# gopro/cineform-sdk

Measured on AMD Instinct MI355X. Metric: 1080p YUY2 encode+decode fps, higher is better.
Workload: dtype int16

## Files before the change

cineform-sdk_amd/csrc/cfhd_kernels.h:

```cpp
#pragma once
#include <stdint.h>
#include <cfhd_gfx950.h>

namespace cfhd {
namespace dev {

enum { TW = 64, TH = 16, ROWS = 2 * TH + 4, NTHREADS = 256, NSTAGE = (ROWS * (TW + 4) + NTHREADS - 1) / NTHREADS };

struct QuantParam { int mid; unsigned mult; int divisor; };

struct FwdPlaneJob {
	const int16_t *in; int in_pitch;
	int width, height;
	int prescale;
	int16_t *out[4]; int out_pitch;
	QuantParam q[4];
	int xstride, shift, display_height;
	int compand;
	int layout, tail_from;
	const uint16_t *curve;
};
enum FwdLayout { FWD_WORDS16 = 0, FWD_V210_Y = 1, FWD_V210_CR = 2, FWD_V210_CB = 3, FWD_BYTES8_BOTTOM_UP = 4, FWD_BYTES8_TOP_DOWN = 5, FWD_RGB10 = 6, FWD_RGB16_AS_422 = 7,
                 FWD_BYTES8_AS_422_BOTTOM_UP = 8, FWD_BYTES8_AS_422_TOP_DOWN = 9, FWD_BAYER_BYR4 = 10, FWD_BAYER_BYR5 = 11,
                 FWD_AVID_BYTES8 = 12, FWD_AVID_WORDS16 = 13, FWD_AVID_S214 = 14, FWD_AVID_2_8 = 15 };
static_assert(FWD_V210_CB < FWD_BYTES8_BOTTOM_UP && FWD_BYTES8_TOP_DOWN < FWD_RGB10 && FWD_RGB10 < FWD_RGB16_AS_422 && FWD_RGB16_AS_422 < FWD_BYTES8_AS_422_BOTTOM_UP &&
              FWD_BYTES8_AS_422_TOP_DOWN < FWD_BAYER_BYR4 && FWD_BAYER_BYR5 == 11 && FWD_BAYER_BYR5 < FWD_AVID_BYTES8 && FWD_AVID_2_8 == 15,
              "fwd_plane_tile's loader tests the pairs as ranges");

__device__ __forceinline__ uint32_t rgb16_to_yuv_sample(const uint16_t *p, int wpp, int which, int color_space, int x)
{
	const int m[4][10] = { { 2998, 10060, 1016, 64, 1655, 5538, 7193, 7193, 6537, 655 }, { 3490, 11715, 1180, 0, 1917, 6455, 8372, 8372, 7602, 770 },
	                       { 4211, 8258, 1606, 64, 2425, 4768, 7193, 7193, 6029, 1163 }, { 4899, 9617, 1868, 0, 2818, 5554, 8372, 8372, 7012, 1360 } };
	const int cs = color_space & 3;
	if (which == 0) {
		const uint16_t *q = p + (size_t)x * wpp;
		const int y = ((m[cs][0] * (int)q[0] + m[cs][1] * (int)q[1] + m[cs][2] * (int)q[2]) >> 20) + m[cs][3];
		return (uint32_t)(y < 0 ? 0 : (y > 1023 ? 1023 : y));
	}
	int acc = 0;
#pragma unroll
	for (int k = 0; k < 2; k++) {
		const uint16_t *q = p + (size_t)(2 * x + k) * wpp;
		const int r = q[0], g = q[1], b = q[2];
		acc += which == 2 ? (-m[cs][4] * r - m[cs][5] * g + m[cs][6] * b) >> 20 : (m[cs][7] * r - m[cs][8] * g - m[cs][9] * b) >> 20;
	}
	acc = (acc >> 1) + 512;
	return (uint32_t)(acc < 0 ? 0 : (acc > 1023 ? 1023 : acc));
}

__device__ __forceinline__ uint32_t rgb8_to_yuv_sample(const uint8_t *row, int bpp, int which, int color_space, int x)
{
	const int m[4][9] = { { 1499, 5029, 507, 827, 2768, 3596, 3596, 3268, 327 }, { 1744, 5857, 589, 958, 3227, 4186, 4186, 3801, 385 },
	                      { 2105, 4128, 802, 1212, 2383, 3596, 3596, 3014, 581 }, { 2449, 4808, 933, 1409, 2777, 4186, 4186, 3506, 679 } };
	const int cs = color_space & 3;
	const uint8_t *q = row + (size_t)(which ? 2 * x : x) * bpp;
	const int b = (int)q[0] << 7, g = (int)q[1] << 7, r = (int)q[2] << 7;
	int v;
	if (which == 0) v = ((((m[cs][0] * r) >> 16) + ((m[cs][1] * g) >> 16) + ((m[cs][2] * b) >> 16)) << 2) + ((cs & 1) ? 0 : 1024);
	else if (which == 2) v = ((((-m[cs][3] * r) >> 16) + ((-m[cs][4] * g) >> 16) + ((m[cs][5] * b) >> 16)) * 4) + 8192;
	else v = ((((m[cs][6] * r) >> 16) + ((-m[cs][7] * g) >> 16) + ((-m[cs][8] * b) >> 16)) * 4) + 8192;
	v = v < 0 ? 0 : (v > 16383 ? 16383 : v);
	return (uint32_t)v >> 4;
}

__device__ __forceinline__ uint32_t bayer_plane_sample(const FwdPlaneJob &job, int row, int x)
{
	int tl, tr, bl, br;
	if (job.layout == FWD_BAYER_BYR5) {
		const uint8_t *base = (const uint8_t *)job.in + (size_t)row * job.width * 6, *nib = base + (size_t)job.width * 4;
		int v[4];
#pragma unroll
		for (int k = 0; k < 4; k++) { const int s = k * job.width + x; v[k] = ((int)base[s] << 4) | ((nib[s >> 1] >> (4 * (s & 1))) & 15); }
		tl = v[0]; tr = v[1]; bl = v[2]; br = v[3];
	} else {
		const uint16_t *l1 = (const uint16_t *)job.in + (size_t)(2 * row) * job.in_pitch, *l2 = l1 + job.in_pitch;
		const uint32_t a = *(const uint32_t *)(l1 + 2 * x), b = *(const uint32_t *)(l2 + 2 * x);
		tl = job.curve[(a & 0xffffu) >> 2]; tr = job.curve[a >> 18]; bl = job.curve[(b & 0xffffu) >> 2]; br = job.curve[b >> 18];
	}
	int r, g1, g2, bb;
	switch (job.xstride) {
	case 0: r = tl; g1 = tr; g2 = bl; bb = br; break;
	case 1: g1 = tl; r = tr; bb = bl; g2 = br; break;
	case 3: bb = tl; g1 = tr; g2 = bl; r = br; break;
	default: g1 = tl; bb = tr; r = bl; g2 = br; break;
	}
	const int mid = 1 << (job.shift - 1), g = (g1 + g2) >> 1;
	const int v = job.tail_from == 0 ? g : (job.tail_from == 1 ? ((r - g) >> 1) + mid : (job.tail_from == 2 ? ((bb - g) >> 1) + mid : (g1 - g2 + 2 * mid) >> 1));
	return (uint32_t)(uint16_t)v;
}

__device__ __forceinline__ uint32_t avid_sample(const FwdPlaneJob &job, int y, int s)
{
	const uint8_t *frame = (const uint8_t *)job.in;
	if (job.layout == FWD_AVID_BYTES8) return (uint32_t)frame[(size_t)y * job.in_pitch + s] << 2;
	if (job.layout == FWD_AVID_2_8) {
		const uint32_t upper = frame[(size_t)y * (job.in_pitch >> 2) + (s >> 2)], lower = frame[(size_t)job.shift + (size_t)y * job.in_pitch + s];
		return (lower << 2) | ((upper >> (6 - 2 * (s & 3))) & 3u);
	}
	const uint32_t w = *(const uint16_t *)(frame + (size_t)y * job.in_pitch + 2 * (size_t)s);
	if (job.layout == FWD_AVID_WORDS16) return w >> 6;
	const int v = (int)(int16_t)w;
	const int n = job.tail_from == 1 ? 219 * v : 224 * (v + 8192);
	const int q = (((n + ((n >> 31) & 16383)) >> 14) + 16) * 4;
	return (uint32_t)(q < 0 ? 0 : (q > 1023 ? 1023 : q));
}

enum { FWD_CHUNK_BLOCKS = 62, FWD_CHUNK_COLS = FWD_CHUNK_BLOCKS * 8 };
struct FwdBlockLists {
	uint4 *blocks;
	unsigned long long *masks;
	const int16_t *base;
	int mask_base[3][4];
	int reserved[2];
};

struct FwdYuvJob {
	const uint8_t *in; int in_pitch;
	int width, height, display_height;
	int uyvy, shift;
	int16_t *out[3][4]; int out_pitch[3];
	QuantParam q[3][4];
	FwdBlockLists lists;
};

struct InvPlaneJob {
	const int16_t *band[4]; int band_pitch;
	int width, height;
	int descale;
	int16_t *out; int out_pitch;
	int xstride, precision, display_height;
	int alpha;
	int alpha_const;
	int bytes8, bottom_up;
	uint32_t dither_seed;
	int bit_shift, big_endian;
	int ll_bottom_row_high;
};

struct InvYuvJob {
	const int16_t *band[3][4]; int band_pitch[3];
	int width, height;
	int display_height;
	int uyvy, shift;
	uint32_t dither_seed;
	uint8_t *out; int out_pitch;
	int bottom_up, matrix_601;
	const unsigned long long *masks; int mask_base[3][4];
};

struct HalfYuvJob {
	const int16_t *ll[3]; int pitch[3];
	int width, rows;
	int uyvy;
	uint8_t *out; int out_pitch;
	int matrix;
	int mode, bottom_up;
};

struct HalfPackedJob {
	const int16_t *ll[4]; int pitch;
	int width, rows, nch;
	int word[4];
	int shift, alpha;
	uint16_t *out; int out_pitch;
	int mode, bytes, bottom_up, big_endian; uint32_t dither_seed;
};

struct FwdFrameJob {
	const uint8_t *in; int in_pitch;
	int width, height, display_height;
	int uyvy, shift;
	int16_t *out[3][4]; int out_pitch[3];
	QuantParam q[3][4];
	FwdBlockLists lists;
};

struct BayerJob {
	const uint16_t *in; int in_pitch;
	int width, height, display_height;
	int16_t *out[4]; int out_pitch;
	const uint16_t *curve;
	int order;
	int precision;
	int packed12;
};

__device__ __forceinline__ int sat16(int x) { return x < -32768 ? -32768 : (x > 32767 ? 32767 : x); }
__device__ __forceinline__ int adds16(int a, int b) { return sat16(a + b); }
__device__ __forceinline__ int subs16(int a, int b) { return sat16(a - b); }
__device__ __forceinline__ int lo16(uint32_t v) { return (int)(int16_t)(v & 0xffffu); }
__device__ __forceinline__ int hi16(uint32_t v) { return (int)(int16_t)(v >> 16); }
__device__ __forceinline__ uint32_t pack16(int lo, int hi) { return ((uint32_t)(uint16_t)lo) | ((uint32_t)(uint16_t)hi << 16); }

__device__ __forceinline__ uint32_t pk_set(int v) { return pack16(v, v); }
__device__ __forceinline__ uint32_t pk_hp_mid(uint32_t a0, uint32_t a1, uint32_t a2, uint32_t a3, uint32_t a4, uint32_t a5)
{
	uint32_t s = pk_subs(0u, a0);
	s = pk_subs(s, a1);
	s = pk_adds(s, a4);
	s = pk_adds(s, a5);
	s = pk_adds(s, pk_set(4));
	s = pk_sra(s, 3);
	return pk_adds(s, pk_subs(a2, a3));
}

__device__ __forceinline__ int quantize(int v, const QuantParam &q)
{
	if (q.divisor <= 1) return v;
	int neg = v < 0;
	unsigned a = ((unsigned)(neg ? -v : v) + (unsigned)q.mid) & 0xffffu;
	int r = (int)((a * (q.mult & 0xffffu)) >> 16);
	return (int)(int16_t)(neg ? -r : r);
}

__device__ __forceinline__ uint32_t pk_quantize(uint32_t v, const QuantParam &q)
{
	if (q.divisor <= 1) return v;
	const uint32_t s = pk_sra(v, 15);
	uint32_t a = pk_maxs(v, pk_negw(v));
	a = pk_addw(a, pk_set(q.mid));
	const uint32_t m = q.mult & 0xffffu;
	const uint32_t r = pk_hihi((a & 0xffffu) * m, (a >> 16) * m);
	return pk_addw(r ^ s, pk_negw(s));
}

__device__ __forceinline__ QuantParam wave_uniform_quant(const QuantParam &q) { QuantParam u; u.mid = wave_uniform(q.mid); u.mult = (unsigned)wave_uniform((int)q.mult); u.divisor = wave_uniform(q.divisor); return u; }

__device__ __forceinline__ int hp_mid(int a0, int a1, int a2, int a3, int a4, int a5)
{
	int s = subs16(0, a0);
	s = subs16(s, a1);
	s = adds16(s, a4);
	s = adds16(s, a5);
	s = adds16(s, 4);
	s >>= 3;
	return adds16(s, subs16(a2, a3));
}
__device__ __forceinline__ int hp_first(int a0, int a1, int a2, int a3, int a4, int a5) { return sat16((5 * a0 - 11 * a1 + 4 * a2 + 4 * a3 - a4 - a5 + 4) >> 3); }
__device__ __forceinline__ int hp_last(int a0, int a1, int a2, int a3, int a4, int a5) { return sat16((11 * a4 - 5 * a5 - 4 * a3 - 4 * a2 + a1 + a0 + 4) >> 3); }

__device__ __forceinline__ void horiz_pair(const uint32_t *d, uint32_t dm2, int prescale, bool first0, bool last0, bool last1, uint32_t &lpk, uint32_t &hpk)
{
	uint32_t p0 = d[0], p1 = d[1], p2 = d[2], p3 = d[3];
	if (prescale) {
		const uint32_t three = pk_set(3);
		p0 = pk_adds(p0, three); p1 = pk_adds(p1, three); p2 = pk_adds(p2, three); p3 = pk_adds(p3, three);
		uint32_t low = pk_adds(pk_lolo(p1, p2), pk_hihi(p1, p2));
		low = pk_subs(low, three);
		lpk = pk_sra(low, 2);
		p0 = pk_sra(p0, 2); p1 = pk_sra(p1, 2); p2 = pk_sra(p2, 2); p3 = pk_sra(p3, 2);
	} else {
		lpk = pk_adds(pk_lolo(p1, p2), pk_hihi(p1, p2));
	}
	const uint32_t em = pk_lolo(p0, p1), om = pk_hihi(p0, p1), e0 = pk_lolo(p1, p2), o0 = pk_hihi(p1, p2), ep = pk_lolo(p2, p3), op = pk_hihi(p2, p3);
	hpk = pk_hp_mid(em, om, e0, o0, ep, op);
	if (first0 || last0 || last1) {
		int h0 = lo16(hpk), h1 = hi16(hpk);
		if (first0) h0 = hp_first(lo16(p1), hi16(p1), lo16(p2), hi16(p2), lo16(p3), hi16(p3));
		if (last0) {
			uint32_t pm = dm2;
			if (prescale) pm = pk_sra(pk_adds(pm, pk_set(3)), 2);
			h0 = hp_last(lo16(pm), hi16(pm), lo16(p0), hi16(p0), lo16(p1), hi16(p1));
		}
		if (last1) h1 = hp_last(lo16(p0), hi16(p0), lo16(p1), hi16(p1), lo16(p2), hi16(p2));
		hpk = pack16(h0, h1);
	}
}

__device__ __forceinline__ void vert_pair_store(const uint32_t *sl, const uint32_t *sh, int stride, int pos, const QuantParam *q,
                                                int16_t *const *out, int out_pitch, int r, int c, bool valid1)
{
	uint32_t L[6], H[6];
#pragma unroll
	for (int k = 0; k < 6; k++) { L[k] = sl[k * stride]; H[k] = sh[k * stride]; }
	uint32_t ll, hl, lh, hh;
	if (pos == 1) {
		ll = pk_adds(L[2], L[3]); hl = pk_hp_mid(L[0], L[1], L[2], L[3], L[4], L[5]);
		lh = pk_adds(H[2], H[3]); hh = pk_hp_mid(H[0], H[1], H[2], H[3], H[4], H[5]);
	} else {
		int res[4][2];
#pragma unroll
		for (int e = 0; e < 2; e++) {
			int a[6], b[6];
#pragma unroll
			for (int k = 0; k < 6; k++) { a[k] = e ? hi16(L[k]) : lo16(L[k]); b[k] = e ? hi16(H[k]) : lo16(H[k]); }
			if (pos == 0) {
				res[0][e] = sat16(a[0] + a[1]); res[2][e] = hp_first(a[0], a[1], a[2], a[3], a[4], a[5]);
				res[1][e] = sat16(b[0] + b[1]); res[3][e] = hp_first(b[0], b[1], b[2], b[3], b[4], b[5]);
			} else {
				res[0][e] = sat16(a[4] + a[5]); res[2][e] = hp_last(a[0], a[1], a[2], a[3], a[4], a[5]);
				res[1][e] = sat16(b[4] + b[5]); res[3][e] = hp_last(b[0], b[1], b[2], b[3], b[4], b[5]);
			}
		}
		ll = pack16(res[0][0], res[0][1]); lh = pack16(res[1][0], res[1][1]); hl = pack16(res[2][0], res[2][1]); hh = pack16(res[3][0], res[3][1]);
	}
	lh = pack16(quantize(lo16(lh), q[1]), quantize(hi16(lh), q[1]));
	hl = pack16(quantize(lo16(hl), q[2]), quantize(hi16(hl), q[2]));
	hh = pack16(quantize(lo16(hh), q[3]), quantize(hi16(hh), q[3]));
	if (!valid1) { ll &= 0xffffu; lh &= 0xffffu; hl &= 0xffffu; hh &= 0xffffu; }
	const size_t o = (size_t)r * out_pitch + c;
	*(uint32_t *)(out[0] + o) = ll; *(uint32_t *)(out[1] + o) = lh; *(uint32_t *)(out[2] + o) = hl; *(uint32_t *)(out[3] + o) = hh;
}

template <typename J> __device__ __forceinline__ void stage_job(J *dst, const J *src)
{
// ... 766 lines not shown
	const int seg_first = tile.x * SSEG;
	const int base = luma ? seg_first + SLUMA_STEP * wave : seg_first >> 1;
	const int want = base - 1 + lane;
	const int blk = want < 0 ? 0 : (want < nblk ? want : nblk - 1);
	const bool stores = lane >= 1 && lane <= SLUMA_STEP && want < nblk;
	const int v_base = SSEG * 4, u_base = v_base + SSEG * 2;
	const int lds_at = luma ? 4 * (want - seg_first) : (comp == 1 ? v_base : u_base) + 4 * (want - (seg_first >> 1));
	const int seg_blocks = job.width / SBLK - seg_first < SSEG ? job.width / SBLK - seg_first : SSEG;
	const int nquads = 2 * seg_blocks;
	const bool first = blk == 0, last = blk == nblk - 1;
	const int pitch = job.band_pitch[comp];
	const int16_t *const bLL = wave_uniform_ptr(job.band[comp][0]), *const bLH = wave_uniform_ptr(job.band[comp][1]);
	const int16_t *const bHL = wave_uniform_ptr(job.band[comp][2]), *const bHH = wave_uniform_ptr(job.band[comp][3]);
	const uint32_t boff = (uint32_t)(SBLK * blk);
#define pLL (bLL + boff)
#define pLH (bLH + boff)
#define pHL (bHL + boff)
#define pHH (bHH + boff)
	if (r0 >= h) return;
	const int nrows = h - r0 < ROWS_PER_STRIP ? h - r0 : ROWS_PER_STRIP;
	int j = inv_window_first_row(r0, h);
	const unsigned long long *const mLH = BLOCKS ? wave_uniform_ptr(job.masks + job.mask_base[comp][1]) : nullptr;
	const unsigned long long *const mHL = BLOCKS ? wave_uniform_ptr(job.masks + job.mask_base[comp][2]) : nullptr;
	const unsigned long long *const mHH = BLOCKS ? wave_uniform_ptr(job.masks + job.mask_base[comp][3]) : nullptr;
	const uint32_t pitch8 = (uint32_t)pitch / SBLK;
#define LOAD_LH(row) (BLOCKS ? strip_load_listed(bLH, mLH, (uint32_t)(row) * pitch8 + (uint32_t)blk) : strip_load(pLH + (size_t)(row) * pitch))
#define LOAD_HL(row) (BLOCKS ? strip_load_listed(bHL, mHL, (uint32_t)(row) * pitch8 + (uint32_t)blk) : strip_load(pHL + (size_t)(row) * pitch))
#define LOAD_HH(row) (BLOCKS ? strip_load_listed(bHH, mHH, (uint32_t)(row) * pitch8 + (uint32_t)blk) : strip_load(pHH + (size_t)(row) * pitch))
	StripRow ll0 = strip_load(pLL + (size_t)j * pitch), ll1 = strip_load(pLL + (size_t)(j + 1) * pitch), ll2 = strip_load(pLL + (size_t)(j + 2) * pitch);
	StripRow lh0 = LOAD_LH(j), lh1 = LOAD_LH(j + 1), lh2 = LOAD_LH(j + 2);
	StripRow hl = LOAD_HL(r0), hh = LOAD_HH(r0);
	const int sh = job.shift;
	uint8_t *const out_base = wave_uniform_ptr(job.out);
	const int out_pitch = wave_uniform(job.out_pitch), display_height = wave_uniform(job.display_height), uyvy = wave_uniform(job.uyvy);
	const int dgroup = luma ? (blk & ~1) : 2 * blk + 1;
	const uint32_t drot = (luma ? (blk & 1) != 0 : comp == 2) ? 8u : 0u;
	for (int s = 0; s < nrows; s++) {
		const int r = r0 + s;
		const bool more = s + 1 < nrows;
		const int jn = more ? inv_window_first_row(r + 1, h) : j;
		const bool advance = jn != j;
		StripRow nll = ll2, nlh = lh2, nhl = hl, nhh = hh;
		if (!LATE_LOADS) {
			if (advance) { nll = strip_load(pLL + (size_t)(jn + 2) * pitch); nlh = LOAD_LH(jn + 2); }
			if (more) { nhl = LOAD_HL(r + 1); nhh = LOAD_HH(r + 1); }
		}
		const int pos = r == 0 ? 0 : (r == h - 1 ? 2 : 1);
		uint32_t Lv[2][4], Hv[2][4];
		if (pos == 1) {
#pragma unroll
			for (int d = 0; d < 4; d++) {
				inv_vert_pk(ll0.d[d], ll1.d[d], ll2.d[d], hl.d[d], 1, Lv[0][d], Lv[1][d]);
				inv_vert_pk(lh0.d[d], lh1.d[d], lh2.d[d], hh.d[d], 1, Hv[0][d], Hv[1][d]);
			}
		} else {
#pragma unroll
			for (int d = 0; d < 4; d++) {
				inv_vert_pk(ll0.d[d], ll1.d[d], ll2.d[d], hl.d[d], pos, Lv[0][d], Lv[1][d]);
				inv_vert_pk(lh0.d[d], lh1.d[d], lh2.d[d], hh.d[d], pos, Hv[0][d], Hv[1][d]);
			}
		}
		uint32_t (*rowbuf)[SROW / 4] = s_rows[s & 1];
#pragma unroll
		for (int par = 0; par < 2; par++) {
			const int orow = 2 * r + par;
			const uint32_t prev = __shfl(Lv[par][3], lane - 1), next = __shfl(Lv[par][0], lane + 1);
			const uint32_t X = sh >= 2 ? rotr32(dither_word(seed, orow, dgroup), drot) : 0u;
			uint32_t out[4];
			strip_row_to8(Lv[par], Hv[par], prev, next, first, last, sh + 1, X, out);
			if (stores) {
				uint32_t *dst = &rowbuf[par][lds_at];
#pragma unroll
				for (int d = 0; d < 4; d++) dst[d] = out[d];
			}
		}
		__syncthreads();
		if (tid < nquads) {
#pragma unroll
			for (int par = 0; par < 2; par++) {
				const int orow = 2 * r + par;
				if (orow >= display_height) continue;
				const uint32_t *row = rowbuf[par];
				const uint32_t y0 = row[2 * tid], y1 = row[2 * tid + 1], vv = row[v_base + tid], uu = row[u_base + tid];
				const uint32_t uv01 = byte_perm(vv, uu, 0x05010400u), uv23 = byte_perm(vv, uu, 0x07030602u);
				uint4 q;
				if (uyvy) {
					q.x = byte_perm(uv01, y0, 0x01050004u); q.y = byte_perm(uv01, y0, 0x03070206u);
					q.z = byte_perm(uv23, y1, 0x01050004u); q.w = byte_perm(uv23, y1, 0x03070206u);
				} else {
					q.x = byte_perm(uv01, y0, 0x05010400u); q.y = byte_perm(uv01, y0, 0x07030602u);
					q.z = byte_perm(uv23, y1, 0x05010400u); q.w = byte_perm(uv23, y1, 0x07030602u);
				}
				*(uint4 *)(out_base + (size_t)orow * out_pitch + 32 * (size_t)seg_first + 16 * (size_t)tid) = q;
			}
		}
		if (LATE_LOADS) {
			if (advance) { nll = strip_load(pLL + (size_t)(jn + 2) * pitch); nlh = LOAD_LH(jn + 2); }
			if (more) { nhl = LOAD_HL(r + 1); nhh = LOAD_HH(r + 1); }
		}
		if (advance) { ll0 = ll1; ll1 = ll2; ll2 = nll; lh0 = lh1; lh1 = lh2; lh2 = nlh; j = jn; }
		hl = nhl; hh = nhh;
	}
#undef pLL
#undef pLH
#undef pHL
#undef pHH
#undef LOAD_LH
#undef LOAD_HL
#undef LOAD_HH
}
__global__ void __launch_bounds__(NTHREADS) k_inv_yuv422_strip(const InvYuvJob *jobs, uint32_t launch_seed) { inv_yuv422_strip<SR, true>(jobs, launch_seed); }
__global__ void __launch_bounds__(NTHREADS) k_inv_yuv422_strip_blocks(const InvYuvJob *jobs, uint32_t launch_seed) { inv_yuv422_strip<SR, true, true>(jobs, launch_seed); }

enum { SRF = 32, SFPLANE = 512 };

__device__ __forceinline__ void strip_fwd_row(const uint32_t (&p)[8], uint32_t prev, uint32_t next, bool first, bool last, uint32_t (&L)[4], uint32_t (&H)[4], int prescale = 0)
{
	const uint32_t ext[10] = { prev, p[0], p[1], p[2], p[3], p[4], p[5], p[6], p[7], next };
#pragma unroll
	for (int m = 0; m < 4; m++) horiz_pair(&ext[2 * m], 0u, prescale, first && m == 0, false, last && m == 3, L[m], H[m]);
}

enum { FWD_LATE_LOADS = 2 };
struct FwdStrip {
	uint32_t LW[6][4], HW[6][4];
	cfhd_u4 raw[2][2];
};

__device__ __forceinline__ void strip_fwd_fetch(FwdStrip &st, const FwdYuvJob &job, const uint8_t *in, int y)
{
#pragma unroll
	for (int k = 0; k < 2; k++) {
		if (y + k < job.display_height) { const uint8_t *p = in + (size_t)(y + k) * job.in_pitch; st.raw[k][0] = CFHD_LDG128(p); st.raw[k][1] = CFHD_LDG128(p + 16); }
		else { cfhd_u4 g; g.x = g.y = g.z = g.w = 0x80808080u; st.raw[k][0] = g; st.raw[k][1] = g; }
	}
}

template <int SLOT>
__device__ __forceinline__ void strip_fwd_push(FwdStrip &st, const FwdYuvJob &job, const uint8_t *in, uint32_t (*buf)[2][SFPLANE], int y, bool prefetch,
                                               bool luma, int comp, int lds_write_at, int lds_read_at, int lane, bool first, bool last, int shift, int ysh0, uint32_t usel, uint32_t vsel)
{
	uint32_t p[2][8];
	if (luma) {
		if (FWD_LATE_LOADS == 2) strip_fwd_fetch(st, job, in, y);
		uint32_t a[2][8];
#pragma unroll
		for (int k = 0; k < 2; k++) {
			a[k][0] = st.raw[k][0].x; a[k][1] = st.raw[k][0].y; a[k][2] = st.raw[k][0].z; a[k][3] = st.raw[k][0].w;
			a[k][4] = st.raw[k][1].x; a[k][5] = st.raw[k][1].y; a[k][6] = st.raw[k][1].z; a[k][7] = st.raw[k][1].w;
		}
		if (prefetch && !FWD_LATE_LOADS) strip_fwd_fetch(st, job, in, y + 2);
#pragma unroll
		for (int k = 0; k < 2; k++) {
#pragma unroll
			for (int i = 0; i < 8; i++) p[k][i] = ((a[k][i] >> ysh0) & 0x00ff00ffu) << shift;
			if (lds_write_at >= 0) {
#pragma unroll
				for (int i = 0; i < 4; i++) {
					buf[k][0][lds_write_at + i] = byte_perm(a[k][2 * i + 1], a[k][2 * i], vsel) << shift;
					buf[k][1][lds_write_at + i] = byte_perm(a[k][2 * i + 1], a[k][2 * i], usel) << shift;
				}
			}
		}
	}
	__syncthreads();
	if (!luma) {
#pragma unroll
		for (int k = 0; k < 2; k++) {
#pragma unroll
			for (int i = 0; i < 8; i++) p[k][i] = buf[k][comp - 1][lds_read_at + i < 0 ? 0 : lds_read_at + i];
		}
	}
#pragma unroll
	for (int k = 0; k < 2; k++) {
		const uint32_t prev = __shfl(p[k][7], lane - 1), next = __shfl(p[k][0], lane + 1);
		strip_fwd_row(p[k], prev, next, first, last, st.LW[SLOT + k], st.HW[SLOT + k]);
	}
	if (luma && prefetch && FWD_LATE_LOADS == 1) strip_fwd_fetch(st, job, in, y + 2);
}

template <int ROWS_PER_STRIP, bool BLOCKS = false, bool DENSE = true>
__device__ __forceinline__ void fwd_yuv422_strip(const FwdYuvJob *jobs)
{
	const TileId tile = xcd_tile();
	__shared__ FwdYuvJob s_job;
	stage_job(&s_job, &jobs[tile.z]);
	const FwdYuvJob &job = s_job;
	__shared__ uint32_t s_pairs[2][2][2][SFPLANE];
	const int W = job.width, H = job.height, HH = H >> 1;
	const int r0 = tile.y * ROWS_PER_STRIP;
	const int tid = threadIdx.x, wave = tid >> 6, lane = tid & 63;
	const bool luma = wave < 2;
	const int comp = luma ? 0 : wave - 1;
	const QuantParam q_lh = wave_uniform_quant(job.q[comp][1]), q_hl = wave_uniform_quant(job.q[comp][2]), q_hh = wave_uniform_quant(job.q[comp][3]);
	const int nblk = luma ? W / 16 : W / 32;
	const int seg_first = tile.x * SSEG;
	const int base = luma ? seg_first + SLUMA_STEP * wave : seg_first >> 1;
	const int want = base - 1 + lane;
	const int blk = want < 0 ? 0 : (want < nblk ? want : nblk - 1);
	const bool stores = lane >= 1 && lane <= SLUMA_STEP && want < nblk;
	const bool first = blk == 0, last = blk == nblk - 1;
	const int lds_write_at = (luma && want >= 0 && want < nblk && (wave == 0 ? lane <= SLUMA_STEP : lane >= 1)) ? 4 * (want - seg_first + 1) : -1;
	const int lds_read_at = 8 * lane - 4;
	if (r0 >= HH) return;
	const int r1 = r0 + ROWS_PER_STRIP < HH ? r0 + ROWS_PER_STRIP : HH;
	const int shift = job.shift;
	const int ysh0 = job.uyvy ? 8 : 0, ub = job.uyvy ? 0 : 1, vb = job.uyvy ? 2 : 3;
	const uint32_t usel = (uint32_t)ub | 0x0c00u | ((uint32_t)(4 + ub) << 16) | 0x0c000000u;
	const uint32_t vsel = (uint32_t)vb | 0x0c00u | ((uint32_t)(4 + vb) << 16) | 0x0c000000u;
	const uint8_t *in = job.in + 32 * (size_t)blk;
	static_assert(SLUMA_STEP == FWD_CHUNK_BLOCKS, "a chunk is what one wave stores of a band row");
	const int chunks_per_row = BLOCKS ? wave_uniform((nblk + FWD_CHUNK_BLOCKS - 1) / FWD_CHUNK_BLOCKS) : 0, chunk = BLOCKS ? wave_uniform(base / FWD_CHUNK_BLOCKS) : 0;
	uint4 *slot0[3]; unsigned long long *mask0[3];
	const int opitch = wave_uniform(job.out_pitch[comp]), pitch8 = opitch >> 3;
	int16_t *outp[4];
#pragma unroll
	for (int b = 0; b < 4; b++) outp[b] = wave_uniform_ptr(job.out[comp][b]);
	if (BLOCKS) {
#pragma unroll
		for (int b = 1; b < 4; b++) {
			slot0[b - 1] = wave_uniform_ptr(job.lists.blocks + (size_t)(job.out[comp][b] - job.lists.base) / 8 + (size_t)(FWD_CHUNK_BLOCKS * chunk));
			mask0[b - 1] = wave_uniform_ptr(job.lists.masks + job.lists.mask_base[comp][b] + chunk);
		}
	}
	FwdStrip st;
	int wtop = window_first_row(r0, HH, H);
	const int lastrow = window_first_row(r1 - 1, HH, H) + 5;
	int t = 0;
#define CFHD_PUSH(SLOT, Y) strip_fwd_push<SLOT>(st, job, in, s_pairs[t & 1], (Y), (Y) + 2 <= lastrow, luma, comp, lds_write_at, lds_read_at, lane, first, last, shift, ysh0, usel, vsel); t++
	if (luma && FWD_LATE_LOADS != 2) strip_fwd_fetch(st, job, in, wtop);
	CFHD_PUSH(0, wtop); CFHD_PUSH(2, wtop + 2); CFHD_PUSH(4, wtop + 4);
	auto band_row = [&](const int r, const int pos) {
		uint32_t o[4][4];
#pragma unroll
		for (int d = 0; d < 4; d++) {
			uint32_t ll, lh, hl, hh;
			if (pos == 1) {
				ll = pk_adds(st.LW[2][d], st.LW[3][d]); hl = pk_hp_mid(st.LW[0][d], st.LW[1][d], st.LW[2][d], st.LW[3][d], st.LW[4][d], st.LW[5][d]);
				lh = pk_adds(st.HW[2][d], st.HW[3][d]); hh = pk_hp_mid(st.HW[0][d], st.HW[1][d], st.HW[2][d], st.HW[3][d], st.HW[4][d], st.HW[5][d]);
			} else {
				int res[4][2];
#pragma unroll
				for (int e = 0; e < 2; e++) {
					int a[6], b[6];
#pragma unroll
					for (int k = 0; k < 6; k++) { a[k] = e ? hi16(st.LW[k][d]) : lo16(st.LW[k][d]); b[k] = e ? hi16(st.HW[k][d]) : lo16(st.HW[k][d]); }
					if (pos == 0) {
						res[0][e] = sat16(a[0] + a[1]); res[2][e] = hp_first(a[0], a[1], a[2], a[3], a[4], a[5]);
						res[1][e] = sat16(b[0] + b[1]); res[3][e] = hp_first(b[0], b[1], b[2], b[3], b[4], b[5]);
					} else {
						res[0][e] = sat16(a[4] + a[5]); res[2][e] = hp_last(a[0], a[1], a[2], a[3], a[4], a[5]);
						res[1][e] = sat16(b[4] + b[5]); res[3][e] = hp_last(b[0], b[1], b[2], b[3], b[4], b[5]);
					}
				}
				ll = pack16(res[0][0], res[0][1]); lh = pack16(res[1][0], res[1][1]); hl = pack16(res[2][0], res[2][1]); hh = pack16(res[3][0], res[3][1]);
			}
			o[0][d] = ll; o[1][d] = pk_quantize(lh, q_lh);
			o[2][d] = pk_quantize(hl, q_hl); o[3][d] = pk_quantize(hh, q_hh);
		}
		if (BLOCKS) {
#pragma unroll
			for (int b = 1; b < 4; b++) {
				const bool nz = stores && (o[b][0] | o[b][1] | o[b][2] | o[b][3]) != 0u;
				const unsigned long long m = __ballot(nz);
				uint4 *rowslots = wave_uniform_ptr(slot0[b - 1] + (size_t)(r * pitch8));
				if (nz) store_u32x4_global(rowslots + wave_mbcnt(m), o[b][0], o[b][1], o[b][2], o[b][3]);
				if (lane == 0 && chunk < chunks_per_row) mask0[b - 1][r * chunks_per_row] = m >> 1;
			}
		}
		if (stores) {
#pragma unroll
			for (int b = 0; b < 4; b++) {
				if (b && BLOCKS && !DENSE) continue;
				store_u32x4_global(outp[b] + (uint32_t)(r * opitch + SBLK * blk), o[b][0], o[b][1], o[b][2], o[b][3]);
			}
		}
	};
	auto window_down = [&]() {
#pragma unroll
		for (int k = 0; k < 4; k++) {
#pragma unroll
			for (int d = 0; d < 4; d++) { st.LW[k][d] = st.LW[k + 2][d]; st.HW[k][d] = st.HW[k + 2][d]; }
		}
	};
	auto any_row = [&](const int r) {
		const int need = window_first_row(r, HH, H);
		if (need != wtop) { window_down(); wtop = need; CFHD_PUSH(4, wtop + 4); }
		band_row(r, r == 0 ? 0 : (r == HH - 1 ? 2 : 1));
	};
	int r = r0;
	for (; r < r1 && (r == r0 || r < 2); r++) any_row(r);
	const int mid_end = r1 < HH - 1 ? r1 : HH - 1;
#define CFHD_MID_ROW(R) window_down(); wtop += 2; CFHD_PUSH(4, wtop + 4); band_row((R), 1)
	for (; r + 3 <= mid_end; r += 3) { CFHD_MID_ROW(r); CFHD_MID_ROW(r + 1); CFHD_MID_ROW(r + 2); }
	for (; r < mid_end; r++) { CFHD_MID_ROW(r); }
#undef CFHD_MID_ROW
	for (; r < r1; r++) any_row(r);
#undef CFHD_PUSH
}
__global__ void __launch_bounds__(NTHREADS) k_fwd_yuv422_strip(const FwdYuvJob *jobs) { fwd_yuv422_strip<SRF>(jobs); }
__global__ void __launch_bounds__(NTHREADS) __attribute__((amdgpu_waves_per_eu(4, 4))) k_fwd_yuv422_strip_blocks(const FwdYuvJob *jobs) { fwd_yuv422_strip<SRF, true, false>(jobs); }
__global__ void __launch_bounds__(NTHREADS) k_fwd_yuv422_strip_blocks_dense(const FwdYuvJob *jobs) { fwd_yuv422_strip<SRF, true, true>(jobs); }

enum { SRP = 16 };

struct StripWho { int job; int blk; bool stores; int strip; };
enum { PLSTEP = 62 };
__device__ __forceinline__ StripWho strip_who(int nframes, int nch, int c0, int nc, int glog, int nstrips, int nblk, bool *wave_idle, int nseg = 1)
{
	const int lane = threadIdx.x & 63, gwave = (int)blockIdx.x * (NTHREADS / 64) + (int)(threadIdx.x >> 6);
	const bool segments = nseg > 1;
	const int per_wave = segments ? 1 : 64 >> glog, sub = segments ? 0 : lane >> glog;
	const int strip = gwave % nstrips, rest = gwave / nstrips, seg = segments ? rest % nseg : 0;
	const int b = segments ? seg * PLSTEP - 1 + lane : (lane & ((1 << glog) - 1));
	const int first_sel = (segments ? rest / nseg : rest) * per_wave, nsel = nframes * nc;
	*wave_idle = first_sel >= nsel;
	int sel = first_sel + sub;
	const bool job_ok = sel < nsel;
	if (!job_ok) sel = nsel - 1;
	StripWho w;
	w.job = (sel / nc) * nch + c0 + sel % nc;
	w.stores = job_ok && b >= 0 && b < nblk && (!segments || (lane >= 1 && lane <= PLSTEP));
	w.blk = b < 0 ? 0 : (b < nblk ? b : nblk - 1);
	w.strip = strip;
	return w;
}

__global__ void __launch_bounds__(NTHREADS) k_inv_plane_strip(const InvPlaneJob *jobs, int nframes, int nch, int c0, int nc, int glog, int nstrips, int w, int h, int nseg)
{
	const int lane = threadIdx.x & 63;
	const int nblk = w / SBLK;
	bool idle;
	const StripWho who = strip_who(nframes, nch, c0, nc, glog, nstrips, nblk, &idle, nseg);
	if (idle) return;
	const InvPlaneJob *job = &jobs[who.job];
	const int blk = who.blk, pitch = job->band_pitch, descale = job->descale;
	const bool first = blk == 0, last = blk == nblk - 1;
	const int16_t *pLL = job->band[0] + SBLK * blk, *pLH = job->band[1] + SBLK * blk, *pHL = job->band[2] + SBLK * blk, *pHH = job->band[3] + SBLK * blk;
	int16_t *out = job->out + 2 * SBLK * blk;
	const int out_pitch = job->out_pitch;
	const int r0 = who.strip * SRP;
	const int nrows = h - r0 < SRP ? h - r0 : SRP;
	int j = inv_window_first_row(r0, h);
	StripRow ll0 = strip_load(pLL + (size_t)j * pitch), ll1 = strip_load(pLL + (size_t)(j + 1) * pitch), ll2 = strip_load(pLL + (size_t)(j + 2) * pitch);
	StripRow lh0 = strip_load(pLH + (size_t)j * pitch), lh1 = strip_load(pLH + (size_t)(j + 1) * pitch), lh2 = strip_load(pLH + (size_t)(j + 2) * pitch);
	StripRow hl = strip_load(pHL + (size_t)r0 * pitch), hh = strip_load(pHH + (size_t)r0 * pitch);
	for (int s = 0; s < nrows; s++) {
		const int r = r0 + s;
		const bool more = s + 1 < nrows;
		const int jn = more ? inv_window_first_row(r + 1, h) : j;
		const bool advance = jn != j;
		StripRow nll = ll2, nlh = lh2, nhl = hl, nhh = hh;
		const int pos = r == 0 ? 0 : (r == h - 1 ? 2 : 1);
		uint32_t Lv[2][4], Hv[2][4];
		if (pos == 1) {
#pragma unroll
			for (int d = 0; d < 4; d++) {
				inv_vert_pk(ll0.d[d], ll1.d[d], ll2.d[d], hl.d[d], 1, Lv[0][d], Lv[1][d]);
				inv_vert_pk(lh0.d[d], lh1.d[d], lh2.d[d], hh.d[d], 1, Hv[0][d], Hv[1][d]);
			}
		} else {
#pragma unroll
			for (int d = 0; d < 4; d++) {
				inv_vert_pk(ll0.d[d], ll1.d[d], ll2.d[d], hl.d[d], pos, Lv[0][d], Lv[1][d]);
				inv_vert_pk(lh0.d[d], lh1.d[d], lh2.d[d], hh.d[d], pos, Hv[0][d], Hv[1][d]);
			}
		}
#pragma unroll
		for (int par = 0; par < 2; par++) {
			const uint32_t (&L)[4] = Lv[par];
			const uint32_t (&H)[4] = Hv[par];
			const uint32_t prev = __shfl(L[3], lane - 1), next = __shfl(L[0], lane + 1);
			const uint32_t ext[6] = { prev, L[0], L[1], L[2], L[3], next };
			uint32_t o[8];
#pragma unroll
			for (int d = 0; d < 4; d++) {
				const uint32_t dm = ext[d], d0 = ext[d + 1], dp = ext[d + 2];
				uint32_t even, odd;
				inv_horiz_pk((dm >> 16) | (d0 << 16), d0, (d0 >> 16) | (dp << 16), H[d], even, odd);
				if (descale) { even = pk_adds(even, even); odd = pk_adds(odd, odd); }
				else { even = pk_sra(even, 1); odd = pk_sra(odd, 1); }
				o[2 * d] = pk_lolo(even, odd); o[2 * d + 1] = pk_hihi(even, odd);
			}
			if (first) {
				const int l[6] = { 0, 0, lo16(L[0]), hi16(L[0]), lo16(L[1]), hi16(L[1]) };
				int e, od;
				inv_horiz_border(l, 2, lo16(H[0]), 0, e, od);
				if (descale) { e = sat16(e * 2); od = sat16(od * 2); } else { e = sat16(e >> 1); od = sat16(od >> 1); }
				o[0] = pack16(e, od);
			}
			if (last) {
				const int l[6] = { lo16(L[2]), hi16(L[2]), lo16(L[3]), hi16(L[3]), 0, 0 };
				int e, od;
				inv_horiz_border(l, 3, hi16(H[3]), 2, e, od);
				if (descale) { e = sat16(e * 2); od = sat16(od * 2); } else { e = sat16(e >> 1); od = sat16(od >> 1); }
				o[7] = pack16(e, od);
			}
			if (who.stores) {
				uint4 *dst = (uint4 *)(out + (size_t)(2 * r + par) * out_pitch);
				uint4 q0, q1;
				q0.x = o[0]; q0.y = o[1]; q0.z = o[2]; q0.w = o[3]; q1.x = o[4]; q1.y = o[5]; q1.z = o[6]; q1.w = o[7];
				dst[0] = q0; dst[1] = q1;
			}
		}
		if (advance) { nll = strip_load(pLL + (size_t)(jn + 2) * pitch); nlh = strip_load(pLH + (size_t)(jn + 2) * pitch); }
		if (more) { nhl = strip_load(pHL + (size_t)(r + 1) * pitch); nhh = strip_load(pHH + (size_t)(r + 1) * pitch); }
		if (advance) { ll0 = ll1; ll1 = ll2; ll2 = nll; lh0 = lh1; lh1 = lh2; lh2 = nlh; j = jn; }
		hl = nhl; hh = nhh;
	}
}

template <int ND>
__device__ __forceinline__ void strip_fwd_emit(const uint32_t (&LW)[6][ND], const uint32_t (&HW)[6][ND], int pos, const QuantParam &q_lh, const QuantParam &q_hl, const QuantParam &q_hh,
                                               uint32_t (&o)[4][ND])
{
#pragma unroll
	for (int d = 0; d < ND; d++) {
		uint32_t ll, lh, hl, hh;
		if (pos == 1) {
			ll = pk_adds(LW[2][d], LW[3][d]); hl = pk_hp_mid(LW[0][d], LW[1][d], LW[2][d], LW[3][d], LW[4][d], LW[5][d]);
			lh = pk_adds(HW[2][d], HW[3][d]); hh = pk_hp_mid(HW[0][d], HW[1][d], HW[2][d], HW[3][d], HW[4][d], HW[5][d]);
		} else {
			int res[4][2];
#pragma unroll
			for (int e = 0; e < 2; e++) {
				int a[6], b[6];
#pragma unroll
				for (int k = 0; k < 6; k++) { a[k] = e ? hi16(LW[k][d]) : lo16(LW[k][d]); b[k] = e ? hi16(HW[k][d]) : lo16(HW[k][d]); }
				if (pos == 0) {
					res[0][e] = sat16(a[0] + a[1]); res[2][e] = hp_first(a[0], a[1], a[2], a[3], a[4], a[5]);
					res[1][e] = sat16(b[0] + b[1]); res[3][e] = hp_first(b[0], b[1], b[2], b[3], b[4], b[5]);
				} else {
					res[0][e] = sat16(a[4] + a[5]); res[2][e] = hp_last(a[0], a[1], a[2], a[3], a[4], a[5]);
					res[1][e] = sat16(b[4] + b[5]); res[3][e] = hp_last(b[0], b[1], b[2], b[3], b[4], b[5]);
				}
			}
			ll = pack16(res[0][0], res[0][1]); lh = pack16(res[1][0], res[1][1]); hl = pack16(res[2][0], res[2][1]); hh = pack16(res[3][0], res[3][1]);
		}
		o[0][d] = ll; o[1][d] = pk_quantize(lh, q_lh);
		o[2][d] = pk_quantize(hl, q_hl); o[3][d] = pk_quantize(hh, q_hh);
	}
}

template <int SLOT>
__device__ __forceinline__ void strip_plane_push(uint32_t (&LW)[6][4], uint32_t (&HW)[6][4], const int16_t *in, int pitch, int y, int prescale, int lane, bool first, bool last)
{
	cfhd_u4 raw[2][2];
#pragma unroll
	for (int k = 0; k < 2; k++) { const int16_t *p = in + (size_t)(y + k) * pitch; raw[k][0] = CFHD_LDG128(p); raw[k][1] = CFHD_LDG128(p + 8); }
#pragma unroll
	for (int k = 0; k < 2; k++) {
		const uint32_t p[8] = { raw[k][0].x, raw[k][0].y, raw[k][0].z, raw[k][0].w, raw[k][1].x, raw[k][1].y, raw[k][1].z, raw[k][1].w };
		const uint32_t prev = __shfl(p[7], lane - 1), next = __shfl(p[0], lane + 1);
		strip_fwd_row(p, prev, next, first, last, LW[SLOT + k], HW[SLOT + k], prescale);
	}
}

__global__ void __launch_bounds__(NTHREADS) k_fwd_plane_strip(const FwdPlaneJob *jobs, int nframes, int nch, int c0, int nc, int glog, int nstrips, int W, int H, int nseg)
{
	const int lane = threadIdx.x & 63;
	const int nblk = W / (2 * SBLK), HH = H >> 1;
	bool idle;
	const StripWho who = strip_who(nframes, nch, c0, nc, glog, nstrips, nblk, &idle, nseg);
	if (idle) return;
	const FwdPlaneJob *job = &jobs[who.job];
	const int blk = who.blk, pitch = job->in_pitch, prescale = job->prescale, out_pitch = job->out_pitch;
	const bool first = blk == 0, last = blk == nblk - 1;
	const int16_t *in = job->in + 2 * SBLK * blk;
	const QuantParam q_lh = job->q[1], q_hl = job->q[2], q_hh = job->q[3];
	int16_t *const out0 = job->out[0] + SBLK * blk, *const out1 = job->out[1] + SBLK * blk, *const out2 = job->out[2] + SBLK * blk, *const out3 = job->out[3] + SBLK * blk;
	const int r0 = who.strip * SRP, r1 = r0 + SRP < HH ? r0 + SRP : HH;
	uint32_t LW[6][4], HW[6][4];
	int wtop = window_first_row(r0, HH, H);
	strip_plane_push<0>(LW, HW, in, pitch, wtop, prescale, lane, first, last);
	strip_plane_push<2>(LW, HW, in, pitch, wtop + 2, prescale, lane, first, last);
	strip_plane_push<4>(LW, HW, in, pitch, wtop + 4, prescale, lane, first, last);
	for (int r = r0; r < r1; r++) {
		const int need = window_first_row(r, HH, H);
		if (need != wtop) {
#pragma unroll
			for (int k = 0; k < 4; k++) {
#pragma unroll
				for (int d = 0; d < 4; d++) { LW[k][d] = LW[k + 2][d]; HW[k][d] = HW[k + 2][d]; }
			}
			wtop = need;
			strip_plane_push<4>(LW, HW, in, pitch, wtop + 4, prescale, lane, first, last);
		}
		uint32_t o[4][4];
		strip_fwd_emit(LW, HW, r == 0 ? 0 : (r == HH - 1 ? 2 : 1), q_lh, q_hl, q_hh, o);
		if (who.stores) {
			const size_t at = (size_t)r * out_pitch;
			uint4 v;
			v.x = o[0][0]; v.y = o[0][1]; v.z = o[0][2]; v.w = o[0][3]; *(uint4 *)(out0 + at) = v;
			v.x = o[1][0]; v.y = o[1][1]; v.z = o[1][2]; v.w = o[1][3]; *(uint4 *)(out1 + at) = v;
			v.x = o[2][0]; v.y = o[2][1]; v.z = o[2][2]; v.w = o[2][3]; *(uint4 *)(out2 + at) = v;
			v.x = o[3][0]; v.y = o[3][1]; v.z = o[3][2]; v.w = o[3][3]; *(uint4 *)(out3 + at) = v;
		}
	}
}

enum { PSR = 32, PSTEP = 62 };
template <int WPP> __device__ __forceinline__ constexpr int packed16_word(int c) { return WPP == 3 ? (c == 0 ? 1 : (c == 1 ? 0 : 2)) : (c == 0 ? 2 : (c == 1 ? 1 : (c == 2 ? 3 : 0))); }

template <int WPP> struct PxRows { cfhd_u4 v[2][WPP]; };
template <int WPP>
__device__ __forceinline__ void px_fetch(PxRows<WPP> &R, const uint16_t *px, int in_pitch, int y, int display_height)
{
#pragma unroll
	for (int k = 0; k < 2; k++) {
		const int yy = y + k < display_height ? y + k : display_height - 1;
		const uint16_t *p = px + (size_t)yy * in_pitch;
#pragma unroll
		for (int j = 0; j < WPP; j++) R.v[k][j] = CFHD_LDG128(p + 8 * j);
	}
}
template <int WPP>
__device__ __forceinline__ uint32_t px_pair(const uint32_t (&w)[4 * WPP], int m, int word, int shift, bool compand)
{
	uint32_t s[2];
#pragma unroll
	for (int e = 0; e < 2; e++) {
		const int i = (2 * m + e) * WPP + word;
		const uint32_t d = w[i >> 1];
		s[e] = (i & 1) ? d >> (16 + shift) : (d & 0xffffu) >> shift;
		if (compand && s[e] > 0 && s[e] < 4095) s[e] = ((s[e] * 223 + 128) >> 8) + 256;
	}
	return s[0] | (s[1] << 16);
}
template <int WPP, int NCH, int SLOT>
__device__ __forceinline__ void px_push(uint32_t (&LW)[NCH][6][2], uint32_t (&HW)[NCH][6][2], const PxRows<WPP> &R, int shift, bool compand_alpha, int prescale, int lane, bool first, bool last)
{
#pragma unroll
	for (int k = 0; k < 2; k++) {
		uint32_t w[4 * WPP];
#pragma unroll
		for (int j = 0; j < WPP; j++) { w[4 * j] = R.v[k][j].x; w[4 * j + 1] = R.v[k][j].y; w[4 * j + 2] = R.v[k][j].z; w[4 * j + 3] = R.v[k][j].w; }
#pragma unroll
		for (int c = 0; c < NCH; c++) {
			uint32_t ext[6];
#pragma unroll
			for (int m = 0; m < 4; m++) ext[1 + m] = px_pair<WPP>(w, m, packed16_word<WPP>(c), shift, compand_alpha && c == 3);
			ext[0] = __shfl(ext[4], lane - 1); ext[5] = __shfl(ext[1], lane + 1);
#pragma unroll
			for (int m = 0; m < 2; m++) horiz_pair(&ext[2 * m], 0u, prescale, first && m == 0, false, last && m == 1, LW[c][SLOT + k][m], HW[c][SLOT + k][m]);
		}
	}
}

#ifndef CFHD_PX_WAVES
#define CFHD_PX_WAVES 2
#endif
template <int WPP, int NCH>
__global__ void __launch_bounds__(NTHREADS) __attribute__((amdgpu_waves_per_eu(CFHD_PX_WAVES, CFHD_PX_WAVES))) k_fwd_packed16_strip(const FwdPlaneJob *jobs, int nframes, int nseg, int nstrips)
{
	const int lane = threadIdx.x & 63, gwave = (int)blockIdx.x * (NTHREADS / 64) + wave_uniform((int)(threadIdx.x >> 6));
	const int seg = gwave % nseg, strip = (gwave / nseg) % nstrips, frame = gwave / (nseg * nstrips);
	if (frame >= nframes) return;
	const FwdPlaneJob *job = jobs + (size_t)frame * NCH;
	const int W = job->width, H = job->height, HH = H >> 1, nblk = W / 8;
	const int b = seg * PSTEP - 1 + lane;
	const bool stores = b >= 0 && b < nblk && lane >= 1 && lane <= PSTEP;
	const int blk = b < 0 ? 0 : (b >= nblk ? nblk - 1 : b);
	const bool first = blk == 0, last = blk == nblk - 1;
	const int in_pitch = job->in_pitch, shift = job->shift, dh = job->display_height, prescale = job->prescale, out_pitch = job->out_pitch;
	const bool compand_alpha = NCH == 4 && job[NCH - 1].compand;
	const uint16_t *px = (const uint16_t *)job->in - packed16_word<WPP>(0) + (size_t)blk * 8 * WPP;
	const int r0 = strip * PSR, r1 = r0 + PSR < HH ? r0 + PSR : HH;
	QuantParam q[NCH][3];
	int16_t *out[NCH][4];
#pragma unroll
	for (int c = 0; c < NCH; c++) {
#pragma unroll
		for (int k = 0; k < 3; k++) q[c][k] = job[c].q[1 + k];
#pragma unroll
		for (int k = 0; k < 4; k++) out[c][k] = job[c].out[k];
	}
	uint32_t LW[NCH][6][2], HW[NCH][6][2];
	int wtop = window_first_row(r0, HH, H);
	PxRows<WPP> R;
	px_fetch<WPP>(R, px, in_pitch, wtop, dh);
	px_push<WPP, NCH, 0>(LW, HW, R, shift, compand_alpha, prescale, lane, first, last);
	px_fetch<WPP>(R, px, in_pitch, wtop + 2, dh);
	px_push<WPP, NCH, 2>(LW, HW, R, shift, compand_alpha, prescale, lane, first, last);
	px_fetch<WPP>(R, px, in_pitch, wtop + 4, dh);
	px_push<WPP, NCH, 4>(LW, HW, R, shift, compand_alpha, prescale, lane, first, last);
	int fetched = -1;
	for (int r = r0; r < r1; r++) {
		const int need = window_first_row(r, HH, H);
		if (need != wtop) {
			if (fetched != need + 4) px_fetch<WPP>(R, px, in_pitch, need + 4, dh);
#pragma unroll
			for (int c = 0; c < NCH; c++) {
#pragma unroll
				for (int k = 0; k < 4; k++) { LW[c][k][0] = LW[c][k + 2][0]; LW[c][k][1] = LW[c][k + 2][1]; HW[c][k][0] = HW[c][k + 2][0]; HW[c][k][1] = HW[c][k + 2][1]; }
			}
			wtop = need;
			px_push<WPP, NCH, 4>(LW, HW, R, shift, compand_alpha, prescale, lane, first, last);
		}
		if (r + 1 < r1) {
			const int next_need = window_first_row(r + 1, HH, H);
			if (next_need != wtop) { px_fetch<WPP>(R, px, in_pitch, next_need + 4, dh); fetched = next_need + 4; }
		}
		const int pos = r == 0 ? 0 : (r == HH - 1 ? 2 : 1);
		const uint32_t at = ((uint32_t)r * (uint32_t)out_pitch + (uint32_t)blk * 4u) * 2u;
#pragma unroll
		for (int c = 0; c < NCH; c++) {
			uint32_t o[4][2];
			strip_fwd_emit<2>(LW[c], HW[c], pos, q[c][0], q[c][1], q[c][2], o);
			if (stores) {
#pragma unroll
				for (int bnd = 0; bnd < 4; bnd++) { uint2 v; v.x = o[bnd][0]; v.y = o[bnd][1]; *(uint2 *)((char *)out[c][bnd] + at) = v; }
			}
		}
	}
}

struct ByRows { cfhd_u4 v[2][2][2]; };
__device__ __forceinline__ void by_fetch(ByRows &R, const uint16_t *mosaic, int in_pitch, int y, int display_height)
{
#pragma unroll
	for (int k = 0; k < 2; k++) {
		const int yy = y + k < display_height ? y + k : display_height - 1;
		const uint16_t *p = mosaic + (size_t)(2 * yy) * in_pitch;
		R.v[k][0][0] = CFHD_LDG128(p); R.v[k][0][1] = CFHD_LDG128(p + 8);
		R.v[k][1][0] = CFHD_LDG128(p + in_pitch); R.v[k][1][1] = CFHD_LDG128(p + in_pitch + 8);
	}
}
template <int SLOT>
__device__ __forceinline__ void by_push(uint32_t (&LW)[4][6][2], uint32_t (&HW)[4][6][2], const ByRows &R, const uint16_t *s_curve, int order, int mid, int prescale, int lane, bool first, bool last)
{
#pragma unroll
	for (int k = 0; k < 2; k++) {
		const uint32_t top[8] = { R.v[k][0][0].x, R.v[k][0][0].y, R.v[k][0][0].z, R.v[k][0][0].w, R.v[k][0][1].x, R.v[k][0][1].y, R.v[k][0][1].z, R.v[k][0][1].w };
		const uint32_t bot[8] = { R.v[k][1][0].x, R.v[k][1][0].y, R.v[k][1][0].z, R.v[k][1][0].w, R.v[k][1][1].x, R.v[k][1][1].y, R.v[k][1][1].z, R.v[k][1][1].w };
		int o[4][8];
#pragma unroll
		for (int q = 0; q < 8; q++) {
			const int tl = s_curve[(top[q] & 0xffffu) >> 2], tr = s_curve[top[q] >> 18], bl = s_curve[(bot[q] & 0xffffu) >> 2], br = s_curve[bot[q] >> 18];
			int r, g1, g2, bb;
			switch (order) {
			case 0: r = tl; g1 = tr; g2 = bl; bb = br; break;
			case 1: g1 = tl; r = tr; bb = bl; g2 = br; break;
			case 3: bb = tl; g1 = tr; g2 = bl; r = br; break;
			default: g1 = tl; bb = tr; r = bl; g2 = br; break;
			}
			const int g = (g1 + g2) >> 1;
			o[0][q] = g; o[1][q] = ((r - g) >> 1) + mid; o[2][q] = ((bb - g) >> 1) + mid; o[3][q] = (g1 - g2 + 2 * mid) >> 1;
		}
#pragma unroll
		for (int c = 0; c < 4; c++) {
			uint32_t ext[6];
#pragma unroll
			for (int m = 0; m < 4; m++) ext[1 + m] = pack16(o[c][2 * m], o[c][2 * m + 1]);
			ext[0] = __shfl(ext[4], lane - 1); ext[5] = __shfl(ext[1], lane + 1);
#pragma unroll
			for (int m = 0; m < 2; m++) horiz_pair(&ext[2 * m], 0u, prescale, first && m == 0, false, last && m == 1, LW[c][SLOT + k][m], HW[c][SLOT + k][m]);
		}
	}
}

__global__ void __launch_bounds__(NTHREADS) __attribute__((amdgpu_waves_per_eu(CFHD_PX_WAVES, CFHD_PX_WAVES))) k_fwd_bayer_strip(const FwdPlaneJob *jobs, const BayerJob *bayer, int nframes, int nseg, int nstrips)
{
	__shared__ uint16_t s_curve[1 << 14];
	{
		const uint4 *src = (const uint4 *)bayer[0].curve;
		uint4 *dst = (uint4 *)s_curve;
		for (int i = threadIdx.x; i < (1 << 14) * 2 / 16; i += NTHREADS) dst[i] = src[i];
	}
	__syncthreads();
	const int lane = threadIdx.x & 63, gwave = (int)blockIdx.x * (NTHREADS / 64) + wave_uniform((int)(threadIdx.x >> 6));
	const int seg = gwave % nseg, strip = (gwave / nseg) % nstrips, frame = gwave / (nseg * nstrips);
	if (frame >= nframes) return;
	const FwdPlaneJob *job = jobs + (size_t)frame * 4;
	const BayerJob *bj = bayer + frame;
	const int W = job->width, H = job->height, HH = H >> 1, nblk = W / 8;
	const int b = seg * PSTEP - 1 + lane;
	const bool stores = b >= 0 && b < nblk && lane >= 1 && lane <= PSTEP;
	const int blk = b < 0 ? 0 : (b >= nblk ? nblk - 1 : b);
	const bool first = blk == 0, last = blk == nblk - 1;
	const int in_pitch = bj->in_pitch, dh = bj->display_height, order = bj->order, mid = 1 << (bj->precision - 1), prescale = job->prescale, out_pitch = job->out_pitch;
	const uint16_t *px = bj->in + (size_t)blk * 16;
	const int r0 = strip * PSR, r1 = r0 + PSR < HH ? r0 + PSR : HH;
	QuantParam q[4][3];
	int16_t *out[4][4];
#pragma unroll
	for (int c = 0; c < 4; c++) {
#pragma unroll
		for (int k = 0; k < 3; k++) q[c][k] = job[c].q[1 + k];
#pragma unroll
		for (int k = 0; k < 4; k++) out[c][k] = job[c].out[k];
	}
	uint32_t LW[4][6][2], HW[4][6][2];
	int wtop = window_first_row(r0, HH, H);
	ByRows R;
	by_fetch(R, px, in_pitch, wtop, dh);
	by_push<0>(LW, HW, R, s_curve, order, mid, prescale, lane, first, last);
	by_fetch(R, px, in_pitch, wtop + 2, dh);
	by_push<2>(LW, HW, R, s_curve, order, mid, prescale, lane, first, last);
	by_fetch(R, px, in_pitch, wtop + 4, dh);
	by_push<4>(LW, HW, R, s_curve, order, mid, prescale, lane, first, last);
	int fetched = -1;
	for (int r = r0; r < r1; r++) {
		const int need = window_first_row(r, HH, H);
		if (need != wtop) {
			if (fetched != need + 4) by_fetch(R, px, in_pitch, need + 4, dh);
#pragma unroll
			for (int c = 0; c < 4; c++) {
#pragma unroll
				for (int k = 0; k < 4; k++) { LW[c][k][0] = LW[c][k + 2][0]; LW[c][k][1] = LW[c][k + 2][1]; HW[c][k][0] = HW[c][k + 2][0]; HW[c][k][1] = HW[c][k + 2][1]; }
			}
			wtop = need;
// ... 888 lines not shown
```

Baseline: 67950.

## Stream inverse-plane strip band rows through a per-wave LDS ring via global_load_lds

New measurement: 68190 (median of 3 runs). About the same (+0.4%).

```diff
diff --git a/cineform-sdk_amd/csrc/cfhd_kernels.h b/cineform-sdk_amd/csrc/cfhd_kernels.h
--- a/cineform-sdk_amd/csrc/cfhd_kernels.h
+++ b/cineform-sdk_amd/csrc/cfhd_kernels.h
@@ -1,6 +1,7 @@
 #pragma once
 #include <stdint.h>
 #include <cfhd_gfx950.h>
+#include <cfhd_lds_ring.h>
 
 namespace cfhd {
 namespace dev {
@@ -1373,7 +1374,7 @@
 __global__ void __launch_bounds__(NTHREADS) __attribute__((amdgpu_waves_per_eu(4, 4))) k_fwd_yuv422_strip_blocks(const FwdYuvJob *jobs) { fwd_yuv422_strip<SRF, true, false>(jobs); }
 __global__ void __launch_bounds__(NTHREADS) k_fwd_yuv422_strip_blocks_dense(const FwdYuvJob *jobs) { fwd_yuv422_strip<SRF, true, true>(jobs); }
 
-enum { SRP = 16 };
+enum { SRP = 16, PLANE_RING = 2 };
 
 struct StripWho { int job; int blk; bool stores; int strip; };
 enum { PLSTEP = 62 };
@@ -1410,18 +1411,49 @@
 	const int16_t *pLL = job->band[0] + SBLK * blk, *pLH = job->band[1] + SBLK * blk, *pHL = job->band[2] + SBLK * blk, *pHH = job->band[3] + SBLK * blk;
 	int16_t *out = job->out + 2 * SBLK * blk;
 	const int out_pitch = job->out_pitch;
-	const int r0 = who.strip * SRP;
+	const int r0 = wave_uniform(who.strip) * SRP;
 	const int nrows = h - r0 < SRP ? h - r0 : SRP;
-	int j = inv_window_first_row(r0, h);
-	StripRow ll0 = strip_load(pLL + (size_t)j * pitch), ll1 = strip_load(pLL + (size_t)(j + 1) * pitch), ll2 = strip_load(pLL + (size_t)(j + 2) * pitch);
-	StripRow lh0 = strip_load(pLH + (size_t)j * pitch), lh1 = strip_load(pLH + (size_t)(j + 1) * pitch), lh2 = strip_load(pLH + (size_t)(j + 2) * pitch);
-	StripRow hl = strip_load(pHL + (size_t)r0 * pitch), hh = strip_load(pHH + (size_t)r0 * pitch);
+	__shared__ cfhd_u4 s_ring[NTHREADS / 64][PLANE_RING][4 * LDS_PIECE];
+	cfhd_u4 (&ring)[PLANE_RING][4 * LDS_PIECE] = s_ring[wave_uniform((int)(threadIdx.x >> 6))];
+	const int j0 = inv_window_first_row(r0, h);
+	int issued = 0;
+	auto new_row = [&](int s) { return s == 0 || inv_window_first_row(r0 + s, h) != inv_window_first_row(r0 + s - 1, h); };
+	auto issue = [&]() {
+		if (issued > nrows) return;
+		cfhd_u4 *at = ring[issued % PLANE_RING];
+		if (issued == 0) {
+			lds_copy16(pLL + (size_t)j0 * pitch, at); lds_copy16(pLH + (size_t)j0 * pitch, at + LDS_PIECE);
+			lds_copy16(pLL + (size_t)(j0 + 1) * pitch, at + 2 * LDS_PIECE); lds_copy16(pLH + (size_t)(j0 + 1) * pitch, at + 3 * LDS_PIECE);
+		} else {
+			const int s = issued - 1;
+			if (new_row(s)) { const int jj = inv_window_first_row(r0 + s, h) + 2; lds_copy16(pLL + (size_t)jj * pitch, at); lds_copy16(pLH + (size_t)jj * pitch, at + LDS_PIECE); }
+			lds_copy16(pHL + (size_t)(r0 + s) * pitch, at + 2 * LDS_PIECE); lds_copy16(pHH + (size_t)(r0 + s) * pitch, at + 3 * LDS_PIECE);
+		}
+		issued++;
+	};
+	auto take = [&](int q, int rounds_done, cfhd_u4 (&v)[4]) {
+		int after = 4 * (rounds_done < PLANE_RING ? rounds_done : PLANE_RING);
+#pragma unroll
+		for (int k = 1; k < PLANE_RING; k++) if (q + k < issued) after += new_row(q + k - 1) ? 4 : 2;
+		lds_wait(after);
+		lds_read16x2(ring[q % PLANE_RING], v[0], v[1]);
+		lds_read16x2(ring[q % PLANE_RING] + 2 * LDS_PIECE, v[2], v[3]);
+		issue();
+	};
+	auto as_row = [](const cfhd_u4 &v) { StripRow t; t.d[0] = v.x; t.d[1] = v.y; t.d[2] = v.z; t.d[3] = v.w; return t; };
+	CFHD_LDS_RING_HOLD(pLL); CFHD_LDS_RING_HOLD(pLH); CFHD_LDS_RING_HOLD(pHL); CFHD_LDS_RING_HOLD(pHH); CFHD_LDS_RING_HOLD(pitch);
+	CFHD_LDS_RING_HOLD(out); CFHD_LDS_RING_HOLD(out_pitch); CFHD_LDS_RING_HOLD(descale);
+	for (int k = 0; k < PLANE_RING; k++) issue();
+	StripRow ll0, ll1, ll2, lh0, lh1, lh2, hl, hh;
+	{ cfhd_u4 v[4]; take(0, 0, v); ll1 = as_row(v[0]); lh1 = as_row(v[1]); ll2 = as_row(v[2]); lh2 = as_row(v[3]); ll0 = ll1; lh0 = lh1; }
 	for (int s = 0; s < nrows; s++) {
 		const int r = r0 + s;
-		const bool more = s + 1 < nrows;
-		const int jn = more ? inv_window_first_row(r + 1, h) : j;
-		const bool advance = jn != j;
-		StripRow nll = ll2, nlh = lh2, nhl = hl, nhh = hh;
+		{
+			cfhd_u4 v[4];
+			take(s + 1, s, v);
+			if (new_row(s)) { ll0 = ll1; ll1 = ll2; ll2 = as_row(v[0]); lh0 = lh1; lh1 = lh2; lh2 = as_row(v[1]); }
+			hl = as_row(v[2]); hh = as_row(v[3]);
+		}
 		const int pos = r == 0 ? 0 : (r == h - 1 ? 2 : 1);
 		uint32_t Lv[2][4], Hv[2][4];
 		if (pos == 1) {
@@ -1468,16 +1500,10 @@
 				o[7] = pack16(e, od);
 			}
 			if (who.stores) {
-				uint4 *dst = (uint4 *)(out + (size_t)(2 * r + par) * out_pitch);
-				uint4 q0, q1;
-				q0.x = o[0]; q0.y = o[1]; q0.z = o[2]; q0.w = o[3]; q1.x = o[4]; q1.y = o[5]; q1.z = o[6]; q1.w = o[7];
-				dst[0] = q0; dst[1] = q1;
-			}
-		}
-		if (advance) { nll = strip_load(pLL + (size_t)(jn + 2) * pitch); nlh = strip_load(pLH + (size_t)(jn + 2) * pitch); }
-		if (more) { nhl = strip_load(pHL + (size_t)(r + 1) * pitch); nhh = strip_load(pHH + (size_t)(r + 1) * pitch); }
-		if (advance) { ll0 = ll1; ll1 = ll2; ll2 = nll; lh0 = lh1; lh1 = lh2; lh2 = nlh; j = jn; }
-		hl = nhl; hh = nhh;
+				int16_t *dst = out + (size_t)(2 * r + par) * out_pitch;
+				store_u32x4_global(dst, o[0], o[1], o[2], o[3]); store_u32x4_global(dst + 8, o[4], o[5], o[6], o[7]);
+			}
+		}
 	}
 }
 
diff --git a/cineform-sdk_amd/csrc/cfhd_lds_ring.h b/cineform-sdk_amd/csrc/cfhd_lds_ring.h
--- /dev/null
+++ b/cineform-sdk_amd/csrc/cfhd_lds_ring.h
@@ -0,0 +1,37 @@
+#pragma once
+#include <stdint.h>
+#include <hip/hip_runtime.h>
+#include <cfhd_gfx950.h>
+
+namespace cfhd {
+namespace dev {
+
+enum { LDS_PIECE = 64 };
+
+__device__ __forceinline__ void lds_copy16(const void *src, cfhd_u4 *piece)
+{
+	__builtin_amdgcn_global_load_lds((const __attribute__((address_space(1))) void *)src, (__attribute__((address_space(3))) void *)piece, 16, 0, 0);
+}
+
+__device__ __forceinline__ void lds_wait(int n)
+{
+#define CFHD_LDS_WAIT_CASE(k) case k: asm volatile("s_waitcnt vmcnt(" #k ")" ::: "memory"); break;
+	switch (wave_uniform(n)) {
+	CFHD_LDS_WAIT_CASE(1) CFHD_LDS_WAIT_CASE(2) CFHD_LDS_WAIT_CASE(3) CFHD_LDS_WAIT_CASE(4) CFHD_LDS_WAIT_CASE(5)
+	CFHD_LDS_WAIT_CASE(6) CFHD_LDS_WAIT_CASE(7) CFHD_LDS_WAIT_CASE(8) CFHD_LDS_WAIT_CASE(9) CFHD_LDS_WAIT_CASE(10)
+	CFHD_LDS_WAIT_CASE(11) CFHD_LDS_WAIT_CASE(12) CFHD_LDS_WAIT_CASE(13) CFHD_LDS_WAIT_CASE(14) CFHD_LDS_WAIT_CASE(15)
+	default: asm volatile("s_waitcnt vmcnt(0)" ::: "memory"); break;
+	}
+#undef CFHD_LDS_WAIT_CASE
+}
+
+__device__ __forceinline__ void lds_read16x2(const cfhd_u4 *piece, cfhd_u4 &r0, cfhd_u4 &r1)
+{
+	const uint32_t at = (uint32_t)(uintptr_t)(const __attribute__((address_space(3))) cfhd_u4 *)piece + 16u * (threadIdx.x & 63u);
+	asm volatile("ds_read_b128 %0, %2\n\tds_read_b128 %1, %2 offset:1024\n\ts_waitcnt lgkmcnt(0)" : "=&v"(r0), "=&v"(r1) : "v"(at) : "memory");
+}
+
+#define CFHD_LDS_RING_HOLD(x) asm volatile("" :: "v"(x))
+
+}
+}
```
